# Pi-Star-Lab/RESCO

Hardware: AMD Instinct MI355X
Metric: env-steps/sec (higher is better)
Workload: dtype f32; 1 GPU; ingolstadt21 x 4096 lock-step envs per GPU (BASELINE config 3), fixed demand from the map's rou.xml, on-device seeded random policy, Krauss sigma 0.5 + speedFactor dev 0.1; tls_expiry=1, map=ingolstadt21, envs_per_gpu=4096, pipes=2, ticks_per_env_step=10, block_threads=512, lds_bytes_per_env=40896, parallelism=env-batch split x1, no collective on the data path

## Files before the change

### resco_amd/csrc/resco_sim.hip

```cpp
#include <hip/hip_runtime.h>
#include <hip/hip_fp16.h>
#include <stdint.h>
#include <stdio.h>
#include <stdlib.h>
#include <string.h>
#include <math.h>
#include <mutex>
#include <new>
#include <string>
#include <vector>

#include "resco_sim.h"

#define RS_DEV __device__ __forceinline__
#define RS_HD __host__ __device__
#define RS_MEM __device__ __forceinline__
#define RS_G(p) (p)
#define RS_CARVE __host__ __device__ __forceinline__
__device__ __forceinline__ void rs_atomic_min(int32_t *p, int32_t v) { atomicMin(p, v); }
__device__ __forceinline__ void rs_atomic_min(uint32_t *p, uint32_t v) { atomicMin(p, v); }
__device__ __forceinline__ void rs_atomic_max(int32_t *p, int32_t v) { atomicMax(p, v); }
__device__ __forceinline__ void rs_atomic_add(int32_t *p, int32_t v) { atomicAdd(p, v); }
__device__ __forceinline__ int32_t rs_atomic_fetch_add(int32_t *p, int32_t v) { return atomicAdd(p, v); }
__device__ __forceinline__ int32_t rs_wave_ticket(int32_t *p) {
    const unsigned long long m = __ballot(1);
    const int below = (int)__builtin_amdgcn_mbcnt_hi((uint32_t)(m >> 32), __builtin_amdgcn_mbcnt_lo((uint32_t)m, 0u));
    int32_t base = 0;
    if (below == 0) base = atomicAdd(p, (int32_t)__popcll(m));
    return __builtin_amdgcn_readlane(base, __ffsll((long long)m) - 1) + below;
}
__device__ __forceinline__ void rs_wave_add(int32_t *p, int32_t v) {
    for (int m = 32; m > 0; m >>= 1) v += __shfl_xor(v, m);
    if ((threadIdx.x & 63) == 0 && v) atomicAdd(p, v);
}
__device__ __forceinline__ void rs_wave_max(int32_t *p, int32_t v) {
    for (int m = 32; m > 0; m >>= 1) { const int32_t o = __shfl_xor(v, m); v = o > v ? o : v; }
    if ((threadIdx.x & 63) == 0) atomicMax(p, v);
}
__device__ __forceinline__ void rs_atomic_or(uint32_t *p, uint32_t v) { atomicOr(p, v); }
__device__ __forceinline__ uint32_t rs_atomic_fetch_or(uint32_t *p, uint32_t v) { return atomicOr(p, v); }
__device__ __forceinline__ int rs_atomic_inc(int32_t *p) { return atomicAdd(p, 1); }
__device__ __forceinline__ void rs_atomic_and(uint32_t *p, uint32_t v) { atomicAnd(p, v); }
__device__ __forceinline__ uint32_t rs_atomic_cas(uint32_t *p, uint32_t cmp, uint32_t v) { return atomicCAS(p, cmp, v); }
__device__ __forceinline__ int rs_ffsll(unsigned long long x) { return __ffsll(x); }
__device__ __forceinline__ int rs_clzll(unsigned long long x) { return __clzll((long long)x); }
__device__ __forceinline__ int rs_ffs(uint32_t x) { return __ffs((int)x); }
__device__ __forceinline__ int rs_popc(uint32_t x) { return __popc(x); }
__device__ __forceinline__ float rs_int_as_float(int x) { return __int_as_float(x); }
__device__ __forceinline__ int rs_float_as_int(float x) { return __float_as_int(x); }
__device__ __forceinline__ uint16_t rs_f2h(float x) { return __half_as_ushort(__float2half(x)); }

#ifndef RS_IEEE_DIV
__device__ __forceinline__ float rs_div_unscaled(float a, float b) {
    const float r0 = __builtin_amdgcn_rcpf(b);
    const float r1 = __builtin_fmaf(__builtin_fmaf(-b, r0, 1.0f), r0, r0);
    const float q0 = a * r1;
    const float q1 = __builtin_fmaf(__builtin_fmaf(-b, q0, a), r1, q0);
    return __builtin_fmaf(__builtin_fmaf(-b, q1, a), r1, q1);
}
#define RS_DIV(a, b) rs_div_unscaled((a), (b))
#endif
#define RS_OPAQUE_S(x) asm volatile("" : "+s"(x));
#ifndef RS_NARROW_NODE
#define RS_KEEP4(a, b, c, d) asm volatile("" : "+v"(a), "+v"(b), "+v"(c), "+v"(d));
#endif
extern __shared__ __attribute__((aligned(16))) char rs_smem[];
#define RS_SMEM rs_smem

#ifdef RS_STUDY_SECTIONS
__device__ unsigned long long *g_sec_prof;
#define RS_SEC_BEGIN unsigned long long sec_t = wall_clock64();
#define RS_SEC(id) { const unsigned long long sec_1 = wall_clock64(); if (g_sec_prof && (threadIdx.x & 63) == 0 && (blockIdx.x & 15) == 0) atomicAdd(&g_sec_prof[id], (sec_1 - sec_t) + (1ull << 40)); sec_t = wall_clock64(); }
#endif
#ifdef RS_DEVICE_ASSERT
#define RS_ASSERT(c) if (!(c)) rs_atomic_add(&L.sc[SC_STATS + ST_INVARIANT], 1);
#endif
#include "resco_host.h"
#include "resco_policy.h"
#include "resco_frap.h"
#include "resco_ppo.h"
#include "resco_ppo_train.h"
#include "resco_dqn_train.h"

struct StepArgs { KTab T; State G; Out O; Lds L; };
typedef const __attribute__((address_space(4))) StepArgs *StepArgsPtr;

template <bool PROF> struct DevExec {
    int B;
    int wave;
    unsigned long long *prof;
    unsigned long long t0;
    template <class F> __device__ __forceinline__ void phase(int id, F f) {
        int w = wave;
        uint32_t ones = ~0u;
        asm volatile("" : "+s"(w), "+s"(ones));
        int tid = (w << 6) | (int)__builtin_amdgcn_mbcnt_hi(ones, __builtin_amdgcn_mbcnt_lo(ones, 0u));
        asm volatile("" : "+v"(tid));
        f(tid);
        __syncthreads();
        if (PROF && prof) {
            const unsigned long long t1 = wall_clock64();
            if (tid == 0) atomicAdd(&prof[id], t1 - t0);
            t0 = t1;
        }
    }
    __device__ __forceinline__ int wave_of(int) const { return wave; }
    __device__ __forceinline__ int next_chunk(int32_t *ctr, int, int, int) const {
        int c = 0;
        if (__builtin_amdgcn_mbcnt_hi(~0u, __builtin_amdgcn_mbcnt_lo(~0u, 0u)) == 0) c = atomicAdd(ctr, 1);
        return __builtin_amdgcn_readfirstlane(c);
    }
    __device__ __forceinline__ unsigned long long role_begin() const { return (PROF && prof) ? wall_clock64() : 0ull; }
    __device__ __forceinline__ void role_end(int id, unsigned long long start) const {
#ifdef RS_STUDY_SECTIONS
        return;
#endif
        if (PROF && prof && (threadIdx.x & 63) == 0 && (blockIdx.x & 15) == 0) atomicAdd(&prof[id], (wall_clock64() - start) + (1ull << 40));
    }
};
template <int CAP, bool PROF> __device__ __forceinline__ void rs_step_kernel_body(StepArgsPtr Ac, const KParams &P, const int32_t *__restrict__ actions) {
    if ((int)blockIdx.x >= P.n_envs) return;
    const StepArgs *A = (const StepArgs *)Ac;
#ifdef RS_STUDY_SECTIONS
    if (threadIdx.x == 0) g_sec_prof = P.prof;
#endif
    DevExec<PROF> ex{(int)blockDim.x, __builtin_amdgcn_readfirstlane((int)threadIdx.x >> 6), PROF ? P.prof : nullptr, (PROF && P.prof) ? wall_clock64() : 0ull};
    rs_step_body<CAP>(ex, A->L, A->T, A->G, A->O, P, actions, (int)blockIdx.x);
}
template <int CAP>
__global__ void __launch_bounds__(1024, 8)
rs_step_kernel_v64(StepArgsPtr Ac, KParams P, const int32_t *__restrict__ actions) { rs_step_kernel_body<CAP, false>(Ac, P, actions); }
template <int CAP>
__global__ void __launch_bounds__(768, 6)
rs_step_kernel_v80(StepArgsPtr Ac, KParams P, const int32_t *__restrict__ actions) { rs_step_kernel_body<CAP, false>(Ac, P, actions); }
template <int CAP>
__global__ void __launch_bounds__(512, 4)
rs_step_kernel_v128(StepArgsPtr Ac, KParams P, const int32_t *__restrict__ actions) { rs_step_kernel_body<CAP, false>(Ac, P, actions); }
__global__ void __launch_bounds__(768, 6)
rs_step_kernel_prof(StepArgsPtr Ac, KParams P, const int32_t *__restrict__ actions) { rs_step_kernel_body<0, true>(Ac, P, actions); }

__global__ void rs_reset_kernel(KTab T, State G, KParams P) { rs_reset_env(T, G, P, (int)blockIdx.x, (int)threadIdx.x, blockDim.x); }
__global__ void rs_reinit_kernel(KTab T, State G, KParams P) { rs_reinit_env(T, G, P, (int)blockIdx.x, (int)threadIdx.x, blockDim.x); }
__global__ void rs_act_random_kernel(KTab T, KParams P, uint32_t step_key, int32_t *actions) {
    const int i = blockIdx.x * blockDim.x + threadIdx.x;
    if (i < P.n_envs * T.n_signals) actions[i] = rs_random_action(T, P, step_key, i);
}
__global__ void rs_act_maxwave_kernel(KTab T, KParams P, const int32_t *pairs, int n_pairs, const int32_t *valid, const int32_t *order,
                                      int use_pressure, const int32_t *mplight, const int32_t *wave, int32_t *actions) {
    const int i = blockIdx.x * blockDim.x + threadIdx.x;
    if (i < P.n_envs * T.n_signals) actions[i] = rs_maxwave_action(T, pairs, n_pairs, valid, order, use_pressure, mplight, wave, i);
}

enum RegBudget { V64 = 0, V128 = 1, V80 = 2 };
struct rs_sim {
    int device = 0;
    int n_envs = 0, env_base = 0, block = 256;
    int ratio = 1;
    size_t lds = 0;
    KTab K{};
    StepArgs *args = nullptr;
    RegBudget budget = V64;
    State G{};
    Out O{};
    KParams P{};
    uint32_t out_mask = OUT_ALL;
    int32_t *actions = nullptr;
    int32_t *pairs = nullptr, *valid = nullptr, *order = nullptr;
    unsigned long long *prof = nullptr;
    int n_pairs = 0;
    hipStream_t stream = nullptr;
// ... 1027 lines not shown
```

### resco_amd/csrc/resco_step.h

```cpp
#pragma once
#include "resco_tables.h"

struct State {
    char *base;
    size_t nc;
    int32_t *trip_log;
    int32_t *env;
    int32_t *tls;
    long long *stats;
    uint16_t *dep_next;
    uint32_t *mail;
    RS_HD float *pos() const { return (float *)base; }
    RS_HD float *speed() const { return RS_G((float *)(base + 4 * nc)); }
    RS_HD float *accel() const { return RS_G((float *)(base + 8 * nc)); }
    RS_HD float *tloss() const { return RS_G((float *)(base + 12 * nc)); }
    RS_HD float *sf() const { return RS_G((float *)(base + 16 * nc)); }
    RS_HD uint32_t *coop(int par) const { return RS_G((uint32_t *)(base + (par ? 43 : 20) * nc)); }
    RS_HD uint32_t *cooplead(int par) const { return RS_G((uint32_t *)(base + (par ? 47 : 24) * nc)); }
    RS_HD uint16_t *lane() const { return RS_G((uint16_t *)(base + 28 * nc)); }
    RS_HD uint16_t *trip() const { return RS_G((uint16_t *)(base + 30 * nc)); }
    RS_HD uint16_t *cursor() const { return RS_G((uint16_t *)(base + 32 * nc)); }
    RS_HD uint16_t *swait() const { return RS_G((uint16_t *)(base + 34 * nc)); }
    RS_HD uint16_t *rwait() const { return RS_G((uint16_t *)(base + 36 * nc)); }
    RS_HD uint16_t *depart() const { return RS_G((uint16_t *)(base + 38 * nc)); }
// ... 692 lines not shown
    float seen = LR.len - x;
    RS_ASSERT(LONG || found || !(seen < look))
    if (LONG && !found && seen < look) {
        int rq = ax.rq;
        int link = (int)(ax.nlink & 0x7FFF);
        int cur_lane = lane;
        const float bgv = d_brake_gap(v, b);
        for (int hop = 0; hop < RM_MAX_HOPS; ++hop) {
            const bool cur_int = (LR.flags & LF_INTERNAL) != 0;
            if (hop > 0) link = (int)(cache_link(T, LR, cur_lane, rq, k) & 0x7FFF);
            bool stop_here = false;
            LinkRec K;
            if (link == NLINK_NONE) {
                if (!cur_int && T.rsteps()[rq].next_edge == 0xFFFF) break;
                stop_here = true;
            } else {
                K = T.links()[link];
                const int st = tls_state(T, L, K.tls, K.tls_pos);
                if (K.tls != 0xFF && (st == TLS_R || st == TLS_Y) && seen >= bgv) stop_here = true;
                if (!stop_here && !(K.flags & KF_CONT) && ((K.flags & KF_MINOR) || (K.tls != 0xFF && st == TLS_g))) {
                    if (seen > RM_VIS_DIST) stop_here = true;
                    else if (K.foe_cnt > 0 && foe_blocked(T, L, grid, K)) stop_here = true;
                }
            }
            if (stop_here) {
                const float g = seen - RM_STOP_OFFSET;
                tgap = g > 0.0f ? g : 0.0f; tvl = 0.0f; tbl = b;
                have = true;
                break;
            }
            LR = K.dest;
            cur_lane = K.to_lane;
            {
                const float vnl = LR.vmax * sf;
                if (vnl < vfree) {
                    const float vs = d_free_speed(seen, vnl, b);
                    if (vs < vsafe) vsafe = vs;
                }
            }
            const Found od = rearmost_within(L, grid, LR.cell0, lane_cells(L, LR), look - seen + T.maxlen);
            if (od.slot != NIL) {
                const float *vo = L.vtp + od.vt() * VT_COLS;
                tgap = seen + od.pos() - vo[VT_LENGTH] - mingap;
                tvl = od.speed(); tbl = vo[VT_DECEL];
                have = true;
                break;
            }
            if (!cur_int) rq += 1;
            seen += LR.len;
            if (!(seen < look)) break;
        }
    }
    if (LONG) RS_SEC(10)
    if (have) {
        const float vs = d_follow_speed(tgap, tvl, b, tbl, tau);
        if (vs < vsafe) vsafe = vs;
    }
    float vmin_n = v - b; if (vmin_n < 0.0f) vmin_n = 0.0f;
    float vmin_e = v - vt[VT_EMERGENCY]; if (vmin_e < 0.0f) vmin_e = 0.0f;
    const float lo = vsafe > vmin_e ? vsafe : vmin_e;
    const float vmin = vmin_n < lo ? vmin_n : lo;
    float vmax = vfree < vsafe ? vfree : vsafe;
    if (vmax < vmin) vmax = vmin;
    const float sigma = P.sigma >= 0.0f ? P.sigma : vt[VT_SIGMA];
    float vd = vmax;
    if (sigma > 0.0f) {
        const float r = d_u01(d_hash(P.seed, (uint32_t)genv, (uint32_t)k, (uint32_t)t, 0u));
        if (vd < a) vd -= sigma * vd * r; else vd -= sigma * a * r;
        if (vd < 0.0f) vd = 0.0f;
    }
    const float vnext = vd > vmin ? vd : vmin;
    L.vnx[s] = vnext;
#ifdef RS_EMU_DEBUG
    if (s == rs_dbg_slot && (t == rs_dbg_t || rs_dbg_t < 0))
        printf("plan t %d slot %d lane %d x %.3f v %.3f lead %d have %d tgap %.3f tvl %.3f vsafe %.3f vfree %.3f vnext %.3f nlink %x\n", t, s, lane, x, v, lead,
               (int)have, tgap, tvl, vsafe, vfree, vnext, ax.nlink);
#endif
    if (LONG) RS_SEC(3)
    if (x + vnext > LR0.len) flag_mover(L, s, t);
    if (LONG) RS_SEC(15)
    (void)LR;
}

template <bool LONG, class LT> RS_DEV void phase_move(const KTab &T, const LT &L, const Grid &gnew, const State &G, const KParams &P, int env, size_t eo,
                       int t, bool last_tick, bool more, int s, int &active, int &halted, int &top) {
    const Aux ax = L.aux[s];
    const Node me = L.node[s];
    const int k = me.trip;
    int lane = ax.lane;
#ifdef RS_EMU_DEBUG
    {
        static int moved_at[65536];
        if (moved_at[s] == t + 1) { printf("slot %d moved twice in tick %d: fl %x lane %d trip %d\n", s, t, me.fl, lane, k); fflush(stdout); abort(); }
        moved_at[s] = t + 1;
    }
#endif
    LaneRec LR = T.lanes()[lane];
    uint32_t nb = T.notbest()[ax.rq];
    uint32_t kw = 0;
    if (more && (ax.nlink & NLINK_ARR)) kw = link_reg_word(T, ax.nlink);
    const float sfv = sf_of(me.sfq);
    float tl = G.tloss()[eo + s];
    const int sw = ax.swait;
    int swn = sw;
    const float vn = L.vnx[s];
    int rq = ax.rq;
    uint16_t nlink = ax.nlink;
    int link = (int)(nlink & 0x7FFF);
    bool relink = false;
    int side = 0;
    RS_ASSERT(LONG || (!(me.fl & (LCT_LEFT | LCT_RIGHT | LCT_SWAP_LEFT | LCT_SWAP_RIGHT)) && !(me.pos + vn > LR.len)))
    if (LONG && (me.fl & (LCT_LEFT | LCT_RIGHT | LCT_SWAP_LEFT | LCT_SWAP_RIGHT))) {
        if ((me.fl & (LCT_LEFT | LCT_RIGHT)) && !(me.pos + vn > LR.len)) side = (me.fl & LCT_LEFT) ? +1 : -1;
        else if (me.fl & (LCT_SWAP_LEFT | LCT_SWAP_RIGHT)) side = (me.fl & LCT_SWAP_LEFT) ? +1 : -1;
    }
    if (LONG && side) {
        lane += side;
        LR = T.lanes()[lane];
        nlink = cache_link(T, LR, lane, rq, k);
        link = (int)(nlink & 0x7FFF);
        relink = true;
    }
    const float vref = LR.vmax * sfv;
    if (last_tick && (P.out_mask & OUT_VEH_ACCEL)) G.accel()[eo + s] = vn - me.speed;
    if (vn <= RM_HALT_SPEED) {
        if (sw < 65535) swn = sw + 1;
        halted += 1;
        if (G.trip_log) { const int wt = G.wtot()[eo + s]; if (wt < 65535) G.wtot()[eo + s] = (uint16_t)(wt + 1); }
    } else swn = 0;
    if (vref > 0.0f && vn < vref) { tl += RS_DIV(vref - vn, vref); G.tloss()[eo + s] = tl; }
    float x = me.pos + vn;
    bool arrived = false;
    if (LONG) for (int it = 0; it < 16; ++it) {
        if (!(x > LR.len)) break;
        const bool li = (LR.flags & LF_INTERNAL) != 0;
        if (link == NLINK_NONE) {
            if (!li && T.rsteps()[rq].next_edge == 0xFFFF) arrived = true; else x = LR.len;
            break;
        }
        x -= LR.len;
        if (!li) rq += 1;
        {
            const LinkRec Km = T.links()[link];
            lane = Km.to_lane;
            LR = Km.dest;
        }
        nlink = cache_link(T, LR, lane, rq, k);
        link = (int)(nlink & 0x7FFF);
        relink = true;
    }
    if (LONG && arrived) {
        Aux na = ax; na.lane = LANE_NONE; na.swait = 0;
        L.aux[s] = na;
        L.node[s].trip = TRIP_NONE; L.node[s].fl = (uint8_t)(me.fl & fl_mh(t));
        rs_atomic_and(&L.alive[s >> 5], ~(1u << (s & 31)));
        {
            const int ow = G.owner()[eo + s];
            if (ow != (int)OWNER_NONE) rs_atomic_add(&L.sig_dep[ow], 1);
        }
        G.owner()[eo + s] = OWNER_NONE; G.rwait()[eo + s] = 0;
        rs_atomic_add(&L.sc[SC_NACT], -1);
        rs_atomic_add(&L.sc[SC_STATS + ST_ARRIVED], 1);
        rs_atomic_add(&L.sc[SC_STATS + ST_DURATION], t + 1 - (int)G.depart()[eo + s]);
        rs_atomic_add(&L.sc[SC_STATS + ST_TLOSS], (int)(tl * 1024.0f + 0.5f));
        if (G.trip_log) {
            int32_t *r = G.trip_log + ((size_t)env * T.n_trips + k) * 4;
            r[0] = (int)G.depart()[eo + s]; r[1] = t + 1; r[2] = (int)(tl * 1024.0f + 0.5f); r[3] = (int)G.wtot()[eo + s];
        }
        return;
    }
    active += 1;
    if (s + 1 > top) top = s + 1;
    Aux na = ax;
    na.lane = (uint16_t)lane; na.rq = (uint16_t)rq; na.swait = (uint16_t)swn;
    if (LONG && relink) na.nlink = nlink;
    L.aux[s] = na;
    Node nn = me;
    nn.pos = x; nn.speed = vn; nn.fl = (uint8_t)(me.fl & fl_mh(t));
    nn.nxt = grid_push(gnew, LR.cell0 + cell_of(L, x, lane_cells(L, LR)), s, vn > RM_HALT_SPEED);
    if (more) {
        if (LONG && relink) { nb = T.notbest()[rq]; if (na.nlink & NLINK_ARR) kw = link_reg_word(T, na.nlink); }
        nn.fl |= classify(T, L, s, L.vtp + me.vt * VT_COLS, vn, x, LR, lane, rq, nb, k, sfv, t + 1);
        L.node[s] = nn;
        if ((na.nlink & NLINK_ARR) && vn > RM_HALT_SPEED) register_approach_w(T, L, kw, vn, x, LR.len, me.vt);
    } else L.node[s] = nn;
    (void)P;
}

template <class LT> RS_DEV int overlapping(const LT &L, const Grid &grid, int cell0, int ncell, float pos, int k, int self, float len_self) {
    const int lead = leader_within(L, grid, cell0, ncell, pos, k, self, RM_NB_WINDOW);
    if (lead != NIL && L.node[lead].pos - L.vtp[L.node[lead].vt * VT_COLS + VT_LENGTH] - pos < 0.0f) return lead;
    const int foll = follower_within(L, grid, cell0, ncell, pos, k, self, RM_NB_WINDOW);
    if (foll != NIL && pos - len_self - L.node[foll].pos < 0.0f) return foll;
    return NIL;
}

template <class LT> RS_DEV int phase_lc_decide(const KTab &T, const LT &L, const Grid &grid, const State &G, size_t eo, int t, int s, const Aux &ax, const Node &me) {
    const int lane = ax.lane;
    const LaneRec LR = T.lanes()[lane];
    const ContRow R = cont_row(T, ax.rq);
    const int my_wait = (int)ax.swait;
    const int n = LR.flags >> 2;
    if ((LR.flags & LF_INTERNAL) || n < 2) return 0;
    const int dir_allowed = (t & 1) ? -1 : +1;
    const int l0 = LR.edge_lane0, kk = lane - l0;
    const int k = me.trip;
    const float *vt = L.vtp + me.vt * VT_COLS;
    const float x = me.pos, v = me.speed;
    const int nc = lane_cells(L, LR);
    int want = 0, dir = dir_allowed;
    float rem;
    const int sdir = strategic_dir(R, kk, n, x, v, 0, rem, grid, LR.cell0, nc, T.occ_unit);
    if (sdir != 0) { dir = sdir; want = 2; }
    int code = 0;
    const int tk = kk + dir;
    if (tk >= 0 && tk < n) {
        const int tcell0 = (int)LR.cell0 + dir * nc;
        int lead_t = NIL, foll_t = NIL;
        bool have_t = false;
        if (!want && !((((uint32_t)t >> 1) + (uint32_t)k) & 3u)) {
            float rem_t;
            if (strategic_dir(R, tk, n, x, v, RM_SG_EXTRA_LANES, rem_t, grid, tcell0, nc, T.occ_unit) == 0) {
                const int lead_c = leader_within(L, grid, LR.cell0, nc, x, k, s, RM_NB_WINDOW);
                if (lead_c != NIL) {
                    lead_t = leader_within(L, grid, tcell0, nc, x, k, s, RM_NB_WINDOW);
                    have_t = true;
                    const float gcur = L.node[lead_c].pos - L.vtp[L.node[lead_c].vt * VT_COLS + VT_LENGTH] - x;
                    float gtgt = RM_BIGF;
                    if (lead_t != NIL) gtgt = L.node[lead_t].pos - L.vtp[L.node[lead_t].vt * VT_COLS + VT_LENGTH] - x;
                    if (gcur < v * 3.0f + 15.0f && gtgt > gcur + RM_SG_ADVANTAGE) want = 1;
                }
            }
        }
        if (want) {
            if (!have_t) lead_t = leader_within(L, grid, tcell0, nc, x, k, s, RM_NB_WINDOW);
            foll_t = follower_within(L, grid, tcell0, nc, x, k, s, RM_NB_WINDOW);
            const bool urgent = want == 2 && rem <= RM_URGENT_DIST;
            bool safe = true;
            if (lead_t != NIL) {
                const Node ld = L.node[lead_t];
                const float *vo = L.vtp + ld.vt * VT_COLS;
                const float gap = ld.pos - vo[VT_LENGTH] - x - (urgent ? 0.0f : vt[VT_MINGAP]);
                const float dec = urgent ? vt[VT_EMERGENCY] : vt[VT_DECEL];
                float vb = v - dec; if (vb < 0.0f) vb = 0.0f;
                if (gap < 0.0f || vb > d_follow_speed(gap, ld.speed, vt[VT_DECEL], vo[VT_DECEL], vt[VT_TAU])) safe = false;
            }
            if (safe && foll_t != NIL) {
                const Node fd = L.node[foll_t];
                const float *vo = L.vtp + fd.vt * VT_COLS;
                const float gap = x - vt[VT_LENGTH] - fd.pos - (urgent ? 0.0f : vo[VT_MINGAP]);
                const float dec = urgent ? vo[VT_EMERGENCY] : vo[VT_DECEL];
                float vb = fd.speed - dec; if (vb < 0.0f) vb = 0.0f;
                if (gap < 0.0f || vb > d_follow_speed(gap, v, vo[VT_DECEL], vt[VT_DECEL], vo[VT_TAU])) safe = false;
            }
            if (safe) {
                if (dir == dir_allowed) code = dir > 0 ? LCT_LEFT : LCT_RIGHT;
            } else if (want == 2) {
                if (lead_t != NIL) { G.cooplead(t & 1)[eo + s] = ((uint32_t)L.node[lead_t].trip << 16) | (uint32_t)lead_t; mail_flag_set(L, s, t & 1); }
                const int R = at_or_behind_within(L, grid, tcell0, nc, x - vt[VT_LENGTH], RM_COOP_RANGE);
                if (R != NIL) { rs_atomic_min(&G.coop(t & 1)[eo + R], ((uint32_t)k << 16) | (uint32_t)s); mail_flag_set(L, R, t & 1); }
            }
        }
    }
    if (sdir != 0 && (t % RM_SWAP_EVERY) == 0 && v <= RM_HALT_SPEED && rem <= RM_URGENT_DIST &&
        my_wait >= RM_SWAP_WAIT) {
        const int b = overlapping(L, grid, (int)LR.cell0 + sdir * nc, nc, x, k, s, vt[VT_LENGTH]);
        if (b != NIL) {
            const Node nb = L.node[b];
            float rem_b;
            if (nb.speed <= RM_HALT_SPEED && (int)L.aux[b].swait >= RM_SWAP_WAIT &&
                strategic_dir(cont_row(T, L.aux[b].rq), kk + sdir, n, nb.pos, nb.speed, 0, rem_b, grid, (int)LR.cell0 + sdir * nc, nc, T.occ_unit) == -sdir && rem_b <= RM_URGENT_DIST &&
                overlapping(L, grid, LR.cell0, nc, nb.pos, nb.trip, b, L.vtp[nb.vt * VT_COLS + VT_LENGTH]) == s)
                code |= sdir > 0 ? LCT_SWAP_LEFT : LCT_SWAP_RIGHT;
        }
    }
        return code;
}

template <class LT> RS_DEV bool phase_insert_decide(const KTab &T, const LT &L, const Grid &grid, int t, int d) {
    if ((int)L.dep_t[d] > t) return false;
    const int k = L.dep[d];
    const DepInfo LR = T.cold.dep_info[d];
    const float *vt = L.vtp + T.trip_vtype()[k] * VT_COLS;
    const float mypos = vt[VT_LENGTH] < LR.len ? vt[VT_LENGTH] : LR.len;
    const int nc = (int)(LR.len * L.cell_inv) + 1;
    const int c1 = LR.cell0 + cell_of(L, mypos + vt[VT_MINGAP] + T.maxlen, nc);
    for (int c = scan_up(grid, LR.cell0, c1); c >= 0; c = (c < c1 ? scan_up(grid, c + 1, c1) : -1))
        for (int o = cell_head(grid, c); o != NIL;) { RS_CHAIN_GUARD
            const Node od = L.node[o];
            const float back = (od.pos + L.vnx[o]) - L.vtp[od.vt * VT_COLS + VT_LENGTH];
            if (back - mypos - vt[VT_MINGAP] < 0.0f) return false;
            o = od.nxt;
        }
    return true;
}

template <class LT> RS_DEV int nth_free_slot(const LT &L, int C, int r) {
#pragma unroll 1
    for (int w = 0; w < (C + 31) / 32; ++w) {
        uint32_t fr = ~L.alive0[w];
        if (w == (C - 1) / 32 && (C & 31)) fr &= (1u << (C & 31)) - 1u;
        const int c = rs_popc(fr);
        if (r >= c) { r -= c; continue; }
#pragma unroll 1
        for (int j = 0; j < r; ++j) fr &= fr - 1u;
        return w * 32 + rs_ffs(fr) - 1;
    }
    return -1;
}

template <class LT> RS_DEV void lc_decide_and_flag(const KTab &T, const LT &L, const Grid &grid, const State &G, size_t eo, int t, int s) {
    const Aux ax = L.aux[s];
    if (ax.lane == LANE_NONE) return;
    const int code = phase_lc_decide(T, L, grid, G, eo, t, s, ax, L.node[s]);
    if (code) flag_mover(L, s, t, code);
}
struct ExecInline {};

template <int CAP, class Exec, class LT>
RS_DEV void rs_step_body_on(Exec &ex, const LT &L, const KTab &T, const State &G, const Out &O, const KParams &P,
                            const int32_t *actions, int env) {
    const int B = ex.B;
    const int C = CAP ? CAP : T.capacity, S = T.n_signals, NO = T.n_obs;
    const int genv = P.env_base + env;
    const size_t eo = (size_t)env * C;
    const int n_ticks = P.n_ticks;

    uint16_t *const grid0 = L.grid;

    ex.phase(0, [&](int tid) {
        if (tid < SC_STATS + ST_N) L.sc[tid] = tid < 4 ? G.env[env * 4 + tid] : 0;
        for (int i = tid; i < T.n_vtypes * VT_COLS; i += B) L.vtp[i] = T.cold.vtype_params[i];
        for (int i = tid; i < (int)(L.gstride >> 1); i += B) ((uint32_t *)grid0)[i] = 0x07FF07FFu;
        for (int i = tid; i < T.n_arr; i += B) L.arr[i] = ARR_NONE;
        for (int i = tid; i < (C + 31) / 32; i += B) { L.alive[i] = 0u; L.mailw[i] = 0u; }
        for (int i = tid; i < (T.n_dep + 31) / 32; i += B) L.insm[i] = 0u;
        for (int i = tid; i < T.n_dep; i += B) {
            const int k = G.dep_next[(size_t)env * T.n_dep + i];
            L.dep[i] = (uint16_t)k;
            L.dep_t[i] = k == (int)TRIP_NONE ? (uint16_t)0xFFFF : (uint16_t)T.cold.trip_depart[k];
        }
        for (int i = tid; i < S; i += B) {
            const int ph = G.tls[(env * S + i) * TLS_W + 0];
            L.phase[i] = ph;
            L.left[i] = G.tls[(env * S + i) * TLS_W + 1];
            L.nextp[i] = G.tls[(env * S + i) * TLS_W + 2];
            L.sig_arr[i] = 0; L.sig_dep[i] = G.tls[(env * S + i) * TLS_W + 3];
            tls_refresh(T, L, P, i, ph);
        }
    });
    ex.phase(1, [&](int tid) {
        const int hw0 = L.sc[SC_HW];
        for (int s = tid; s < C; s += B) {
            uint16_t ln = LANE_NONE, tr = TRIP_NONE;
            if (s < hw0) { ln = G.lane()[eo + s]; tr = G.trip()[eo + s]; }
            Aux ax; ax.lane = ln; ax.rq = 0; ax.nlink = NLINK_NONE; ax.swait = 0;
            if (ln == LANE_NONE) { L.aux[s] = ax; L.node[s].trip = TRIP_NONE; continue; }
            const float sp = G.speed()[eo + s], x = G.pos()[eo + s];
            const int rq = (int)T.routes()[T.trip_route()[tr]].start + (int)G.cursor()[eo + s];
            const LaneRec LR0 = T.lanes()[ln];
            ax.rq = (uint16_t)rq;
            ax.nlink = cache_link(T, LR0, ln, rq, tr);
            ax.swait = G.swait()[eo + s];
            L.aux[s] = ax;
            Node nn; nn.pos = x; nn.speed = sp; nn.trip = tr; nn.vt = T.trip_vtype()[tr];
            nn.fl = 0; nn.sfq = (uint16_t)speed_factor_q(P, genv, tr, L.vtp + nn.vt * VT_COLS);
            if ((G.mail[(size_t)env * ((C + 31) / 32) + (s >> 5)] >> (s & 31)) & 1u) nn.sfq |= (uint16_t)SFQ_MAIL((L.sc[SC_T] + 1) & 1);
            nn.nxt = grid_push(Grid{grid0, 0u}, LR0.cell0 + cell_of(L, x, lane_cells(L, LR0)), s, sp > RM_HALT_SPEED);
            if (n_ticks > 0) nn.fl = (uint8_t)classify(T, L, s, L.vtp + nn.vt * VT_COLS, sp, x, LR0, ln, rq, T.notbest()[rq], tr, sf_of(nn.sfq), L.sc[SC_T]);
            L.node[s] = nn;
            rs_atomic_or(&L.alive[s >> 5], 1u << (s & 31));
        }
        for (int s = B - 1 - tid; s < S; s += B) {
            if (P.do_fsm && !P.fixed_program) {
                const int a = actions[env * S + s], cur = L.phase[s], Gn = T.cold.tls_ngreen[s];
                if (a < 0 || a >= T.cold.tls_nphase[s]) L.nextp[s] = cur;
                else {
                    L.nextp[s] = a;
                    if (cur != a && cur < Gn && a < Gn) {
                        const int y = T.cold.tls_yellow[T.cold.tls_yel_off[s] + cur * Gn + a];
                        if (y >= 0) set_phase(T, L, P, s, y);
                    }
                }
            }
            if (n_ticks > 0) tls_begin_of_tick(T, L, P, s, 0);
        }
    });
    if (n_ticks > 0) ex.phase(2, [&](int tid) {
        const int hw = L.sc[SC_HW];
        for (int s = tid; s < hw; s += B) {
            const Aux ax = L.aux[s];
            if (ax.lane == LANE_NONE) continue;
            const Node me = L.node[s];
            register_approach(T, L, ax.nlink, me.speed, me.pos, T.lanes()[ax.lane].len, me.vt);
        }
    });

    int cur = 0;
    for (int tick = 0; tick < n_ticks; ++tick) {
        const int t = L.sc[SC_T], hw = L.sc[cur ? SC_HWNEW : SC_HW];
        const Grid gold{grid0, cur ? CELL_TAG : 0u}, gnew{grid0, cur ? 0u : CELL_TAG};
        const bool more = tick + 1 < n_ticks;
        const int lcap = (int)L.lcap;
        const int nwv = B >> 6;
        ex.phase(4, [&](int tid) {
            const int wv = ex.wave_of(tid), ln = tid & 63;
            const int nh = L.sc[SC_NH], nlc = L.sc[SC_NLC];
            const unsigned long long r0 = ex.role_begin();
            int role = 0;
            if (nh > lcap || nlc > lcap) {
                for (int pass = 0; pass < 2; ++pass)
                    for (int w = tid; w < hw; w += B) {
                        if (pass && !(L.node[w].fl & FL_LC)) continue;
                        if (pass) lc_decide_and_flag(T, L, gold, G, eo, t, w);
                        else phase_plan<true>(T, L, gold, G, eo, P, genv, t, w);
                    }
            } else {
                const int hch = (nh + RS_H_CHUNK - 1) / RS_H_CHUNK, lch = (nlc + RS_LIST_CHUNK - 1) / RS_LIST_CHUNK;
                const int total = hch + lch + ((hw + 63) >> 6);
                for (int it = 0;; ++it) {
                    const int c = ex.next_chunk(&L.sc[SC_CHUNK_P], wv, it, nwv);
                    if (c >= total) break;
                    if (c < hch) {
                        role = 1;
                        const int w = c * RS_H_CHUNK + ln;
                        if (ln < RS_H_CHUNK && w < nh) phase_plan<true>(T, L, gold, G, eo, P, genv, t, L.ls_h[w]);
                    } else if (c < hch + lch) {
                        role = 2;
                        const int w = (c - hch) * RS_LIST_CHUNK + ln;
                        if (ln < RS_LIST_CHUNK && w < nlc) lc_decide_and_flag(T, L, gold, G, eo, t, L.ls_lc[w]);
                    } else {
                        const int w = (c - hch - lch) * 64 + ln;
                        if (w < hw && !(L.node[w].fl & FL_H)) phase_plan<false>(T, L, gold, G, eo, P, genv, t, w);
                    }
                }
            }
            ex.role_end(role == 1 ? 7 : (role == 2 ? 8 : 9), r0);
            for (int i = tid; i < (T.n_dep + 31) / 32; i += B) L.insm[i] = 0u;
        });
        ex.phase(5, [&](int tid) {
            for (int i = tid; i < T.n_arr; i += B) L.arr[i] = ARR_NONE;
            for (int i = tid; i < (C + 31) / 32; i += B) L.alive0[i] = L.alive[i];
            int Bs = B;
            RS_OPAQUE_S(Bs)
            for (int i = tid; i < (int)(L.gstride >> 2); i += Bs) {
                unsigned long long *q = (unsigned long long *)grid0 + i;
                const unsigned long long w = *q;
                const unsigned long long st = ((w ^ grid_tag4(gold)) >> 15) & 0x0001000100010001ull;
                if (st) { const unsigned long long m = st * 0xFFFFull; *q = (w & ~m) | ((0x07FF07FF07FF07FFull | grid_tag4(gold)) & m); }
            }
            for (int d = B - 1 - tid; d < T.n_dep; d += B)
                if (phase_insert_decide(T, L, gold, t, d)) rs_atomic_or(&L.insm[d >> 5], 1u << (d & 31));
            if (more)
                for (int sg = B - 1 - tid; sg < S; sg += B) tls_begin_of_tick(T, L, P, sg, tick + 1);
            if (tid == 0) {
                L.sc[SC_T] = t + 1; L.sc[SC_STATS + ST_TICKS] += 1;
                L.sc[cur ? SC_HW : SC_HWNEW] = 0;
                L.sc[SC_ROOM] = C - L.sc[SC_NACT];
                L.sc[SC_NH] = 0; L.sc[SC_NLC] = 0;
                L.sc[SC_NMH + ((t + 1) & 1)] = 0;
                L.sc[SC_CHUNK_P] = 0; L.sc[SC_CHUNK_M] = 0;
            }
        });
        ex.phase(6, [&](int tid) {
            int active = 0, halted = 0, top = 0;
            const int wv = ex.wave_of(tid), ln = tid & 63;
            const int nmh = L.sc[SC_NMH + (t & 1)];
            int ich = 0;
            for (int i = 0; i < (T.n_dep + 31) / 32; ++i) if (L.insm[i]) ich = 1;
            const bool all = nmh > lcap;
            const int mch = all ? 0 : (nmh + RS_LIST_CHUNK - 1) / RS_LIST_CHUNK;
            const int total = mch + ich + ((hw + 63) >> 6);
            const unsigned long long r0 = ex.role_begin();
            bool list = false;
            for (int it = 0;; ++it) {
                const int c = ex.next_chunk(&L.sc[SC_CHUNK_M], wv, it, nwv);
                if (c >= total) break;
                if (c < mch) {
                    list = true;
                    const int w = c * RS_LIST_CHUNK + ln;
                    if (ln < RS_LIST_CHUNK && w < nmh) phase_move<true>(T, L, gnew, G, P, env, eo, t, !more, more, L.ls_mh[w], active, halted, top);
                } else if (c < mch + ich) {
                    for (int d = 63 - ln; d < T.n_dep; d += 64) {
                        if (!(L.insm[d >> 5] & (1u << (d & 31)))) continue;
                        int rank = rs_popc(L.insm[d >> 5] & ((1u << (d & 31)) - 1u));
                        for (int w = 0; w < (d >> 5); ++w) rank += rs_popc(L.insm[w]);
                        if (rank >= L.sc[SC_ROOM]) { rs_atomic_add(&L.sc[SC_STATS + ST_CAP_BLOCKED], 1); continue; }
                        const int s = nth_free_slot(L, C, rank);
                        if (s < 0) continue;
                        const int k = L.dep[d];
                        const int v = T.trip_vtype()[k];
                        const float *vt = L.vtp + v * VT_COLS;
                        const RouteRec RR = T.routes()[T.trip_route()[k]];
                        const LaneRec LRd = T.lanes()[RR.depart_lane];
                        const int sfq = speed_factor_q(P, genv, k, vt);
                        const float sfn = sf_of(sfq);
                        Node nn; nn.pos = vt[VT_LENGTH] < RR.depart_len ? vt[VT_LENGTH] : RR.depart_len;
                        nn.speed = 0.0f; nn.trip = (uint16_t)k; nn.vt = (uint8_t)v; nn.fl = 0; nn.sfq = (uint16_t)sfq;
                        nn.nxt = grid_push(gnew, LRd.cell0 + cell_of(L, nn.pos, lane_cells(L, LRd)), s, false);
                        if (more) nn.fl = (uint8_t)classify(T, L, s, vt, 0.0f, nn.pos, LRd, RR.depart_lane, (int)RR.start, T.notbest()[RR.start], k, sfn, t + 1);
                        L.node[s] = nn;
                        Aux na; na.lane = RR.depart_lane; na.rq = (uint16_t)RR.start; na.swait = 0;
                        na.nlink = cache_link(T, LRd, RR.depart_lane, (int)RR.start, k);
                        L.aux[s] = na;
                        G.sf()[eo + s] = sfn; G.tloss()[eo + s] = 0.0f; G.cooplead(0)[eo + s] = COOP_NONE; G.cooplead(1)[eo + s] = COOP_NONE; G.coop(0)[eo + s] = COOP_NONE; G.coop(1)[eo + s] = COOP_NONE;
                        G.rwait()[eo + s] = 0; G.owner()[eo + s] = OWNER_NONE; G.depart()[eo + s] = (uint16_t)(t + 1); G.accel()[eo + s] = 0.0f; G.wtot()[eo + s] = 0;
                        {
                            const int k2 = T.cold.trip_next[k];
                            L.dep[d] = (uint16_t)k2;
                            L.dep_t[d] = k2 == (int)TRIP_NONE ? (uint16_t)0xFFFF : (uint16_t)T.cold.trip_depart[k2];
                        }
                        rs_atomic_or(&L.alive[s >> 5], 1u << (s & 31));
                        rs_atomic_add(&L.sc[SC_NACT], 1);
                        rs_atomic_add(&L.sc[SC_NINS], 1);
                        rs_atomic_add(&L.sc[SC_STATS + ST_INSERTED], 1);
                        rs_atomic_add(&L.sc[SC_STATS + ST_DEPDELAY], t - T.cold.trip_depart[k]);
                        if (s + 1 > top) top = s + 1;
                    }
                } else {
                    const int w = (c - mch - ich) * 64 + ln;
                    if (w < hw && (L.alive0[w >> 5] & (1u << (w & 31)))) {
                        if (all) phase_move<true>(T, L, gnew, G, P, env, eo, t, !more, more, w, active, halted, top);
                        else if (!(L.node[w].fl & fl_mh(t))) phase_move<false>(T, L, gnew, G, P, env, eo, t, !more, more, w, active, halted, top);
                    }
                }
            }
            ex.role_end(list ? 10 : 3, r0);
            rs_wave_add(&L.sc[SC_STATS + ST_ACTIVE_TICKS], active);
            rs_wave_add(&L.sc[SC_STATS + ST_WAITING], halted);
            rs_wave_max(&L.sc[cur ? SC_HW : SC_HWNEW], top);
            ex.role_end(15, r0);
        });
        cur ^= 1;
    }
    const int hw_end = L.sc[cur ? SC_HWNEW : SC_HW];

    const bool obs = P.do_observe != 0;
    if (obs) ex.phase(11, [&](int tid) {
        for (int i = tid; i < NO; i += B) { L.agg_q[i] = 0; L.agg_a[i] = 0; L.agg_w[i] = 0; L.agg_m[i] = 0; L.agg_s[i] = 0; L.agg_n[i] = 0; }
    });
    ex.phase(12, [&](int tid) {
        const int hw0 = G.env[env * 4 + 2];
        const int top = hw_end > hw0 ? hw_end : hw0;
        int hi = 0;
        for (int s = tid; s < top; s += B) {
            const int lane = L.aux[s].lane;
            G.lane()[eo + s] = (uint16_t)lane; G.trip()[eo + s] = L.node[s].trip;
            if (lane == (int)LANE_NONE) continue;
            hi = s + 1;
            if (L.node[s].sfq & SFQ_MAIL((L.sc[SC_T] + 1) & 1)) rs_atomic_or(&L.mailw[s >> 5], 1u << (s & 31));
            const int rq = L.aux[s].rq;
            G.pos()[eo + s] = L.node[s].pos; G.speed()[eo + s] = L.node[s].speed; G.swait()[eo + s] = L.aux[s].swait;
            G.cursor()[eo + s] = (uint16_t)(rq - (int)T.routes()[T.trip_route()[L.node[s].trip]].start);
            if (!obs) continue;
            const int prev_owner = G.owner()[eo + s];
            const LaneRec LR = T.lanes()[lane];
            const int oi = T.cold.lane_obs[lane];
            bool detect = false;
            if (oi >= 0) {
                const float d = (LR.len - L.node[s].pos) + T.rsteps()[rq].tlsdist;
                detect = d <= P.max_distance;
            }
            if (!detect) {
                if (prev_owner != (int)OWNER_NONE) rs_atomic_add(&L.sig_dep[prev_owner], 1);
                G.owner()[eo + s] = OWNER_NONE; G.rwait()[eo + s] = 0;
                continue;
            }
            const int sig = T.cold.obs_sig[oi];
            int rw = G.rwait()[eo + s];
            if (prev_owner != sig) {
                rw = 0;
                rs_atomic_add(&L.sig_arr[sig], 1);
                rs_atomic_add(&L.agg_n[oi], 1);
                if (prev_owner != (int)OWNER_NONE) rs_atomic_add(&L.sig_dep[prev_owner], 1);
            }
            if (rw > 0) { rw += T.step_length; if (rw > 65535) rw = 65535; }
            else { const int sw = L.aux[s].swait; if (sw > 0) rw = sw; }
            G.rwait()[eo + s] = (uint16_t)rw;
            G.owner()[eo + s] = (uint8_t)sig;
            if (rw > 0) { rs_atomic_add(&L.agg_q[oi], 1); rs_atomic_add(&L.agg_w[oi], rw); rs_atomic_max(&L.agg_m[oi], rw); }
            else rs_atomic_add(&L.agg_a[oi], 1);
            rs_atomic_add((int32_t *)&L.agg_s[oi], (int32_t)(uint32_t)(L.node[s].speed * 65536.0f + 0.5f));
        }
        if (hi) rs_atomic_max(&L.sc[SC_HWOUT], hi);
    });
    ex.phase(13, [&](int tid) {
        const uint32_t om = obs ? P.out_mask : 0u;
        if (om & (OUT_LANE_AGG | OUT_DRQ_NORM)) for (int i = tid; i < NO * 5; i += B) {
            const int oi = i / 5, c = i - oi * 5;
            const int sg = T.cold.obs_sig[oi];
            const float sp = (float)L.agg_s[oi] * (1.0f / 65536.0f);
            float raw, nrm;
            if (c == 0) { raw = (float)L.agg_q[oi]; nrm = (oi - T.cold.sig_obs_start[sg]) == L.phase[sg] ? 1.0f : 0.0f; }
            else if (c == 1) { raw = (float)L.agg_a[oi]; nrm = raw / 28.0f; }
            else if (c == 2) { raw = (float)L.agg_w[oi]; nrm = raw / 28.0f; }
            else if (c == 3) { raw = (float)L.agg_m[oi]; nrm = (float)L.agg_q[oi] / 28.0f; }
            else { raw = sp; nrm = sp / 20.0f / 28.0f; }
            if (om & OUT_LANE_AGG) O.lane_agg()[(size_t)env * NO * 5 + i] = raw;
            if (om & OUT_DRQ_NORM) O.drq_norm()[(size_t)env * NO * 5 + i] = nrm;
        }
        if (om & OUT_LANE_ARR) for (int i = tid; i < NO; i += B) O.lane_arr()[(size_t)env * NO + i] = L.agg_n[i];
        if (om & OUT_DRQ_F16) for (int i = tid; i < S * T.lmax * 5; i += B) {
            const int sg = i / (T.lmax * 5), r = i - sg * T.lmax * 5;
            const int l = r / 5, c = r - l * 5;
            const int o0 = T.cold.sig_obs_start[sg];
            float nrm = 0.0f;
            if (l < T.cold.sig_obs_start[sg + 1] - o0) {
                const int oi = o0 + l;
                if (c == 0) nrm = l == L.phase[sg] ? 1.0f : 0.0f;
                else if (c == 1) nrm = (float)L.agg_a[oi] / 28.0f;
                else if (c == 2) nrm = (float)L.agg_w[oi] / 28.0f;
                else if (c == 3) nrm = (float)L.agg_q[oi] / 28.0f;
                else nrm = (float)L.agg_s[oi] * (1.0f / 65536.0f) / 20.0f / 28.0f;
            }
            O.drq_f16()[(size_t)env * S * T.lmax * 5 + i] = rs_f2h(nrm);
        }
        if (om & (OUT_MPLIGHT | OUT_WAVE | OUT_MPLIGHT_FULL)) for (int i = tid; i < S * 12; i += B) {
            const int sg = i / 12, m = i - sg * 12;
            int q = 0, wv = 0, tw = 0, ap = 0;
            float last_speed = 0.0f;
            for (int j = T.cold.mv_in_start[i]; j < T.cold.mv_in_start[i + 1]; ++j) {
                const int oi = T.cold.mv_in_idx[j];
                q += L.agg_q[oi]; wv += L.agg_q[oi] + L.agg_a[oi]; tw += L.agg_w[oi]; ap += L.agg_a[oi];
                last_speed = (float)L.agg_s[oi] * (1.0f / 65536.0f);
            }
            for (int j = T.cold.mv_out_start[i]; j < T.cold.mv_out_start[i + 1]; ++j) q -= L.agg_q[T.cold.mv_out_idx[j]];
            const size_t so = (size_t)env * S + sg;
            if (om & OUT_MPLIGHT) O.mplight()[so * 13 + 1 + m] = q;
            if (om & OUT_WAVE) O.wave()[so * 12 + m] = wv;
            if (om & OUT_MPLIGHT_FULL) {
                float *mf = O.mplight_full() + so * 49 + 1 + m * 4;
                mf[0] = (float)q; mf[1] = (float)tw / 28.0f; mf[2] = last_speed; mf[3] = (float)ap / 28.0f;
            }
        }
        for (int sg = tid; sg < S; sg += B) {
            const int ph = L.phase[sg];
            if (obs) {
                const int o0 = T.cold.sig_obs_start[sg], o1 = T.cold.sig_obs_start[sg + 1];
                int tw = 0, tq = 0, mq = 0;
                for (int oi = o0; oi < o1; ++oi) { tw += L.agg_w[oi]; const int qq = L.agg_q[oi]; tq += qq; if (qq > mq) mq = qq; }
                const size_t so = (size_t)env * S + sg;
                O.phase()[so] = ph; O.queue_sum()[so] = tq; O.queue_max()[so] = mq;
                O.wait()[so] = -(float)tw;
                const float wn = -(float)tw / 224.0f;
                O.wait_norm()[so] = wn < -4.0f ? -4.0f : (wn > 4.0f ? 4.0f : wn);
                int pr = tq;
                for (int i = T.cold.pr_out_start[sg]; i < T.cold.pr_out_start[sg + 1]; ++i) pr -= L.agg_q[T.cold.pr_out_idx[i]];
                O.pressure()[so] = -pr;
                if (om & OUT_MPLIGHT) O.mplight()[so * 13] = ph;
                if (om & OUT_MPLIGHT_FULL) O.mplight_full()[so * 49] = (float)ph;
                O.arrivals()[so] = L.sig_arr[sg]; O.departures()[so] = L.sig_dep[sg];
            }
            G.tls[(env * S + sg) * TLS_W + 0] = ph;
            G.tls[(env * S + sg) * TLS_W + 1] = L.left[sg];
            G.tls[(env * S + sg) * TLS_W + 2] = L.nextp[sg];
            G.tls[(env * S + sg) * TLS_W + 3] = obs ? 0 : L.sig_dep[sg];
        }
        for (int i = tid; i < T.n_dep; i += B) G.dep_next[(size_t)env * T.n_dep + i] = L.dep[i];
        for (int i = tid; i < (C + 31) / 32; i += B) G.mail[(size_t)env * ((C + 31) / 32) + i] = L.mailw[i];
    });
    ex.phase(14, [&](int tid) {
        if (tid == 0) {
            G.env[env * 4 + 0] = L.sc[SC_T]; G.env[env * 4 + 1] = L.sc[SC_NINS]; G.env[env * 4 + 3] = L.sc[SC_NACT];
            G.env[env * 4 + 2] = L.sc[SC_HWOUT];
        }
        if (tid < ST_N) {
            long long *st = G.stats + (size_t)env * ST_N;
            if (tid == ST_ACTIVE) st[tid] = L.sc[SC_NACT];
            else if (tid == ST_PENDING) {
                const int t = L.sc[SC_T];
                const int hz = t - 1 <= T.horizon ? t - 1 : T.horizon;
                st[tid] = (t >= 1 ? T.cold.trips_cum[hz] : 0) - L.sc[SC_NINS];
            } else st[tid] += L.sc[SC_STATS + tid];
        }
    });
}

template <int CAP, class Exec>
RS_DEV void rs_step_body(Exec &ex, const Lds &L, const KTab &T, const State &G, const Out &O, const KParams &P,
                         const int32_t *actions, int env) {
    if constexpr (CAP != 0) {
        const LdsFix<CAP> Lf(L);
        rs_step_body_on<CAP>(ex, Lf, T, G, O, P, actions, env);
    } else rs_step_body_on<CAP>(ex, L, T, G, O, P, actions, env);
}
```

Before: 3.878 million env-steps/s.

## Precompute mover lane-walk in prior phase and carry result into move phase

Moves the lane-change and link-following walk for moving vehicles into a separate move_walk function. When the executor keeps thread locals, the walk runs during phase 5 and its result is carried in registers into the move phase, with statically owned list chunks assigned to each wave. The goal is to take the dependent table-lookup chain off the critical path of the move phase. In exchange it adds register pressure, repeats lane-record loads for vmax, and renumbers the final profiling phase id.

```diff
diff --git a/resco_amd/csrc/resco_sim.hip b/resco_amd/csrc/resco_sim.hip
--- a/resco_amd/csrc/resco_sim.hip
+++ b/resco_amd/csrc/resco_sim.hip
@@ -86,6 +86,7 @@
 typedef const __attribute__((address_space(4))) StepArgs *StepArgsPtr;
 
 template <bool PROF> struct DevExec {
+    static constexpr bool keeps_thread_locals = true;
     int B;
     int wave;
     unsigned long long *prof;
diff --git a/resco_amd/csrc/resco_step.h b/resco_amd/csrc/resco_step.h
--- a/resco_amd/csrc/resco_step.h
+++ b/resco_amd/csrc/resco_step.h
@@ -798,46 +798,86 @@
     (void)LR;
 }
 
+struct MovePre {
+    float x;
+    uint32_t lq;
+};
+#define LCT_ANY (LCT_LEFT | LCT_RIGHT | LCT_SWAP_LEFT | LCT_SWAP_RIGHT)
+RS_DEV int move_side(int fl, bool leaves) {
+    if ((fl & (LCT_LEFT | LCT_RIGHT)) && !leaves) return (fl & LCT_LEFT) ? +1 : -1;
+    if (fl & (LCT_SWAP_LEFT | LCT_SWAP_RIGHT)) return (fl & LCT_SWAP_LEFT) ? +1 : -1;
+    return 0;
+}
+RS_DEV bool lane_rec_same(const LaneRec &a, const LaneRec &b) {
+    return a.len == b.len && a.vmax == b.vmax && a.link_start == b.link_start && a.link_cnt == b.link_cnt && a.flags == b.flags && a.cell0 == b.cell0 &&
+           a.edge_lane0 == b.edge_lane0;
+}
+template <class LT> RS_DEV MovePre move_walk(const KTab &T, const LT &L, int s) {
+    const Aux ax = L.aux[s];
+    const Node me = L.node[s];
+    const float vn = L.vnx[s];
+    const int k = me.trip;
+    int lane = ax.lane, rq = ax.rq;
+    LaneRec LR = T.lanes()[lane];
+    int link = (int)(ax.nlink & 0x7FFF);
+    bool have = true;
+    if (me.fl & LCT_ANY) {
+        const int side = move_side(me.fl, me.pos + vn > LR.len);
+        if (side) { lane += side; LR = T.lanes()[lane]; have = false; }
+    }
+    float x = me.pos + vn;
+    for (int it = 0; it < 16; ++it) {
+        if (!(x > LR.len)) break;
+        if (!have) link = (int)(cache_link(T, LR, lane, rq, k) & 0x7FFF);
+        const bool li = (LR.flags & LF_INTERNAL) != 0;
+        if (link == NLINK_NONE) {
+            if (!li && T.rsteps()[rq].next_edge == 0xFFFF) lane = LANE_NONE; else x = LR.len;
+            break;
+        }
+        x -= LR.len;
+        if (!li) rq += 1;
+        const LinkRec Km = T.links()[link];
+        lane = Km.to_lane;
+        LR = Km.dest;
+        RS_ASSERT(lane_rec_same(Km.dest, T.lanes()[Km.to_lane]))
+        have = false;
+    }
+    return MovePre{x, (uint32_t)lane | ((uint32_t)rq << 16)};
+}
 template <bool LONG, class LT> RS_DEV void phase_move(const KTab &T, const LT &L, const Grid &gnew, const State &G, const KParams &P, int env, size_t eo,
-                       int t, bool last_tick, bool more, int s, int &active, int &halted, int &top) {
+                       int t, bool last_tick, bool more, int s, const MovePre pre, int &active, int &halted, int &top) {
     const Aux ax = L.aux[s];
     const Node me = L.node[s];
     const int k = me.trip;
-    int lane = ax.lane;
 #ifdef RS_EMU_DEBUG
     {
         static int moved_at[65536];
-        if (moved_at[s] == t + 1) { printf("slot %d moved twice in tick %d: fl %x lane %d trip %d\n", s, t, me.fl, lane, k); fflush(stdout); abort(); }
+        if (moved_at[s] == t + 1) { printf("slot %d moved twice in tick %d: fl %x lane %d trip %d\n", s, t, me.fl, (int)ax.lane, k); fflush(stdout); abort(); }
         moved_at[s] = t + 1;
     }
 #endif
-    LaneRec LR = T.lanes()[lane];
-    uint32_t nb = T.notbest()[ax.rq];
+    const bool arrived = LONG && (pre.lq & 0xFFFFu) == LANE_NONE;
+    const int lane = (LONG && !arrived) ? (int)(pre.lq & 0xFFFFu) : (int)ax.lane;
+    const int rq = (LONG && !arrived) ? (int)(pre.lq >> 16) : (int)ax.rq;
+    const bool relink = LONG && (lane != (int)ax.lane || rq != (int)ax.rq);
+    const LaneRec LR = T.lanes()[lane];
+    const uint32_t nb = T.notbest()[rq];
+    uint16_t nlink = ax.nlink;
+    if (LONG && relink) nlink = cache_link(T, LR, lane, rq, k);
     uint32_t kw = 0;
-    if (more && (ax.nlink & NLINK_ARR)) kw = link_reg_word(T, ax.nlink);
+    if (more && (nlink & NLINK_ARR)) kw = link_reg_word(T, nlink);
     const float sfv = sf_of(me.sfq);
     float tl = G.tloss()[eo + s];
     const int sw = ax.swait;
     int swn = sw;
     const float vn = L.vnx[s];
-    int rq = ax.rq;
-    uint16_t nlink = ax.nlink;
-    int link = (int)(nlink & 0x7FFF);
-    bool relink = false;
-    int side = 0;
-    RS_ASSERT(LONG || (!(me.fl & (LCT_LEFT | LCT_RIGHT | LCT_SWAP_LEFT | LCT_SWAP_RIGHT)) && !(me.pos + vn > LR.len)))
-    if (LONG && (me.fl & (LCT_LEFT | LCT_RIGHT | LCT_SWAP_LEFT | LCT_SWAP_RIGHT))) {
-        if ((me.fl & (LCT_LEFT | LCT_RIGHT)) && !(me.pos + vn > LR.len)) side = (me.fl & LCT_LEFT) ? +1 : -1;
-        else if (me.fl & (LCT_SWAP_LEFT | LCT_SWAP_RIGHT)) side = (me.fl & LCT_SWAP_LEFT) ? +1 : -1;
-    }
-    if (LONG && side) {
-        lane += side;
-        LR = T.lanes()[lane];
-        nlink = cache_link(T, LR, lane, rq, k);
-        link = (int)(nlink & 0x7FFF);
-        relink = true;
-    }
-    const float vref = LR.vmax * sfv;
+    RS_ASSERT(LONG || (!(me.fl & LCT_ANY) && !(me.pos + vn > LR.len)))
+    float vmax = LONG ? T.lanes()[ax.lane].vmax : LR.vmax;
+    if (LONG && (me.fl & LCT_ANY)) {
+        const int side = move_side(me.fl, me.pos + vn > T.lanes()[ax.lane].len);
+        if (side) vmax = T.lanes()[(int)ax.lane + side].vmax;
+    }
+    const float vref = vmax * sfv;
     if (last_tick && (P.out_mask & OUT_VEH_ACCEL)) G.accel()[eo + s] = vn - me.speed;
     if (vn <= RM_HALT_SPEED) {
         if (sw < 65535) swn = sw + 1;
@@ -845,26 +885,7 @@
         if (G.trip_log) { const int wt = G.wtot()[eo + s]; if (wt < 65535) G.wtot()[eo + s] = (uint16_t)(wt + 1); }
     } else swn = 0;
     if (vref > 0.0f && vn < vref) { tl += RS_DIV(vref - vn, vref); G.tloss()[eo + s] = tl; }
-    float x = me.pos + vn;
-    bool arrived = false;
-    if (LONG) for (int it = 0; it < 16; ++it) {
-        if (!(x > LR.len)) break;
-        const bool li = (LR.flags & LF_INTERNAL) != 0;
-        if (link == NLINK_NONE) {
-            if (!li && T.rsteps()[rq].next_edge == 0xFFFF) arrived = true; else x = LR.len;
-            break;
-        }
-        x -= LR.len;
-        if (!li) rq += 1;
-        {
-            const LinkRec Km = T.links()[link];
-            lane = Km.to_lane;
-            LR = Km.dest;
-        }
-        nlink = cache_link(T, LR, lane, rq, k);
-        link = (int)(nlink & 0x7FFF);
-        relink = true;
-    }
+    const float x = LONG ? pre.x : me.pos + vn;
     if (LONG && arrived) {
         Aux na = ax; na.lane = LANE_NONE; na.swait = 0;
         L.aux[s] = na;
@@ -889,13 +910,12 @@
     if (s + 1 > top) top = s + 1;
     Aux na = ax;
     na.lane = (uint16_t)lane; na.rq = (uint16_t)rq; na.swait = (uint16_t)swn;
-    if (LONG && relink) na.nlink = nlink;
+    na.nlink = nlink;
     L.aux[s] = na;
     Node nn = me;
     nn.pos = x; nn.speed = vn; nn.fl = (uint8_t)(me.fl & fl_mh(t));
     nn.nxt = grid_push(gnew, LR.cell0 + cell_of(L, x, lane_cells(L, LR)), s, vn > RM_HALT_SPEED);
     if (more) {
-        if (LONG && relink) { nb = T.notbest()[rq]; if (na.nlink & NLINK_ARR) kw = link_reg_word(T, na.nlink); }
         nn.fl |= classify(T, L, s, L.vtp + me.vt * VT_COLS, vn, x, LR, lane, rq, nb, k, sfv, t + 1);
         L.node[s] = nn;
         if ((na.nlink & NLINK_ARR) && vn > RM_HALT_SPEED) register_approach_w(T, L, kw, vn, x, LR.len, me.vt);
@@ -1032,6 +1052,8 @@
     if (code) flag_mover(L, s, t, code);
 }
 struct ExecInline {};
+template <class E, class = void> struct exec_keeps_thread_locals { static constexpr bool value = false; };
+template <class E> struct exec_keeps_thread_locals<E, decltype((void)E::keeps_thread_locals)> { static constexpr bool value = E::keeps_thread_locals; };
 
 template <int CAP, class Exec, class LT>
 RS_DEV void rs_step_body_on(Exec &ex, const LT &L, const KTab &T, const State &G, const Out &O, const KParams &P,
@@ -1112,6 +1134,12 @@
         }
     });
 
+#ifdef RS_NO_PREWALK
+    constexpr bool prewalk = false;
+#else
+    constexpr bool prewalk = true;
+#endif
+    constexpr bool carry = prewalk && exec_keeps_thread_locals<Exec>::value;
     int cur = 0;
     for (int tick = 0; tick < n_ticks; ++tick) {
         const int t = L.sc[SC_T], hw = L.sc[cur ? SC_HWNEW : SC_HW];
@@ -1154,7 +1182,15 @@
             ex.role_end(role == 1 ? 7 : (role == 2 ? 8 : 9), r0);
             for (int i = tid; i < (T.n_dep + 31) / 32; i += B) L.insm[i] = 0u;
         });
+        MovePre pre{0.0f, 0u};
         ex.phase(5, [&](int tid) {
+            if constexpr (carry) {
+                const int nmh = L.sc[SC_NMH + (t & 1)];
+                const int w = ex.wave_of(tid) * RS_LIST_CHUNK + (tid & 63);
+                const unsigned long long r0 = ex.role_begin();
+                if (nmh <= lcap && (tid & 63) < RS_LIST_CHUNK && w < nmh) pre = move_walk(T, L, L.ls_mh[w]);
+                if (nmh <= lcap && ex.wave_of(tid) * RS_LIST_CHUNK < nmh) ex.role_end(14, r0);
+            }
             for (int i = tid; i < T.n_arr; i += B) L.arr[i] = ARR_NONE;
             for (int i = tid; i < (C + 31) / 32; i += B) L.alive0[i] = L.alive[i];
             int Bs = B;
@@ -1189,13 +1225,22 @@
             const int total = mch + ich + ((hw + 63) >> 6);
             const unsigned long long r0 = ex.role_begin();
             bool list = false;
+            const int own = prewalk ? (mch < nwv ? mch : nwv) : 0;
+            if (wv < own) {
+                list = true;
+                const int w = wv * RS_LIST_CHUNK + ln;
+                if (ln < RS_LIST_CHUNK && w < nmh) {
+                    const int s = L.ls_mh[w];
+                    phase_move<true>(T, L, gnew, G, P, env, eo, t, !more, more, s, carry ? pre : move_walk(T, L, s), active, halted, top);
+                }
+            }
             for (int it = 0;; ++it) {
-                const int c = ex.next_chunk(&L.sc[SC_CHUNK_M], wv, it, nwv);
+                const int c = own + ex.next_chunk(&L.sc[SC_CHUNK_M], wv, it, nwv);
                 if (c >= total) break;
                 if (c < mch) {
                     list = true;
                     const int w = c * RS_LIST_CHUNK + ln;
-                    if (ln < RS_LIST_CHUNK && w < nmh) phase_move<true>(T, L, gnew, G, P, env, eo, t, !more, more, L.ls_mh[w], active, halted, top);
+                    if (ln < RS_LIST_CHUNK && w < nmh) { const int s = L.ls_mh[w]; phase_move<true>(T, L, gnew, G, P, env, eo, t, !more, more, s, move_walk(T, L, s), active, halted, top); }
                 } else if (c < mch + ich) {
                     for (int d = 63 - ln; d < T.n_dep; d += 64) {
                         if (!(L.insm[d >> 5] & (1u << (d & 31)))) continue;
@@ -1236,8 +1281,8 @@
                 } else {
                     const int w = (c - mch - ich) * 64 + ln;
                     if (w < hw && (L.alive0[w >> 5] & (1u << (w & 31)))) {
-                        if (all) phase_move<true>(T, L, gnew, G, P, env, eo, t, !more, more, w, active, halted, top);
-                        else if (!(L.node[w].fl & fl_mh(t))) phase_move<false>(T, L, gnew, G, P, env, eo, t, !more, more, w, active, halted, top);
+                        if (all) phase_move<true>(T, L, gnew, G, P, env, eo, t, !more, more, w, move_walk(T, L, w), active, halted, top);
+                        else if (!(L.node[w].fl & fl_mh(t))) phase_move<false>(T, L, gnew, G, P, env, eo, t, !more, more, w, MovePre{0.0f, 0u}, active, halted, top);
                     }
                 }
             }
@@ -1375,7 +1420,7 @@
         for (int i = tid; i < T.n_dep; i += B) G.dep_next[(size_t)env * T.n_dep + i] = L.dep[i];
         for (int i = tid; i < (C + 31) / 32; i += B) G.mail[(size_t)env * ((C + 31) / 32) + i] = L.mailw[i];
     });
-    ex.phase(14, [&](int tid) {
+    ex.phase(13, [&](int tid) {
         if (tid == 0) {
             G.env[env * 4 + 0] = L.sc[SC_T]; G.env[env * 4 + 1] = L.sc[SC_NINS]; G.env[env * 4 + 3] = L.sc[SC_NACT];
             G.env[env * 4 + 2] = L.sc[SC_HWOUT];
```

New measurement: 3.855 million env-steps/s. Within noise of the previous version (-0.6%).
